# voidful/DeSTA2.5-Audio

Hardware: AMD Instinct MI355X
Metric: train steps/sec (node) Whisper-v3+Llama3.1-8B Q-Former6L at 1/2/4/8 MI355X (higher is better)
Workload: dtype bf16

## Files before the change

desta2.5-audio_amd/csrc/gemm_bf16.hip:

```cpp
#include "common.h"
#include "desta_hip.h"
#include <math.h>

#ifndef GEMM_GROUP_M
#define GEMM_GROUP_M 8
#endif

namespace {

typedef __attribute__((ext_vector_type(4))) unsigned u32x4;
typedef __attribute__((ext_vector_type(2))) float f32x2;

constexpr int BM = 128, BN = 128, BK = 64;
constexpr int TILE_BYTES = BM * BK * 2;

struct GemmArgs {
    const bf16_t* A; const bf16_t* B; void* C;
    int M, N, K;
    long lda, ldb, ldc;
    long sA, sB, sC;
    const float* bias;
    const void* res; long ldr; long sR; int res_f32;
    int act;
    int out_f32;
    bf16_t* preact; long ldp; long sP;
    float alpha;
    bf16_t* aux; long lda_x;
    unsigned drop_thresh, seed_lo, seed_hi; float drop_scale;
    int tilesM, tilesN;
    int full_tiles, split;
    union {
        float* ws;
        const float* b_scale;
    };
    int* tickets;
    const float* rms_w; float rms_eps;
    const float* rope_cs; const int* rope_pos; int rope_cols, rope_hd;
    int tail_skip;
};

__device__ __forceinline__ void rope4(const GemmArgs& p, int m, int n0, float (&v)[4]) {
    if (p.rope_cs && n0 < p.rope_cols) {
        const int pos = p.rope_pos[m];
        const float4 cs = *(const float4*)(p.rope_cs + ((long)pos * (p.rope_hd >> 1) + ((n0 & (p.rope_hd - 1)) >> 1)) * 2);
        const float a0 = v[0], b0 = v[1], a1 = v[2], b1 = v[3];
        v[0] = a0 * cs.x - b0 * cs.y; v[1] = b0 * cs.x + a0 * cs.y;
        v[2] = a1 * cs.z - b1 * cs.w; v[3] = b1 * cs.z + a1 * cs.w;
    }
}

__device__ __forceinline__ void gelu4_bf16(float (&v)[4]) {
#pragma unroll
    for (int e = 0; e < 4; ++e) v[e] = gelu_erf_fast(v[e]);
}

__device__ __forceinline__ void glds16(const void* g, void* l) {
    __builtin_amdgcn_global_load_lds((const __attribute__((address_space(1))) void*)g,
                                     (__attribute__((address_space(3))) void*)l, 16, 0, 0);
}

template <bool ROPE = false>
__device__ __forceinline__ void epilogue4(const GemmArgs& p, int z, int m, int n0, const f32x4& a) {
    float v[4];
#pragma unroll
    for (int e = 0; e < 4; ++e) v[e] = a[e] * p.alpha;
    if (p.bias) {
        const float4 b = *(const float4*)(p.bias + n0);
        v[0] += b.x; v[1] += b.y; v[2] += b.z; v[3] += b.w;
    }
    if constexpr (ROPE) rope4(p, m, n0, v);
    if (p.preact) {
        u16x4 o;
#pragma unroll
        for (int e = 0; e < 4; ++e) o[e] = f2bf(v[e]);
        *(u16x4*)(p.preact + (long)z * p.sP + (long)m * p.ldp + n0) = o;
    }
    if (p.act == 1) {
        if (p.out_f32) {
#pragma unroll
            for (int e = 0; e < 4; ++e) v[e] = gelu_erf(v[e]);
        } else {
            gelu4_bf16(v);
        }
    }
    if (p.drop_thresh) {
        const unsigned long base = ((unsigned long)z * p.M + m) * p.N + n0;
#pragma unroll
        for (int e = 0; e < 4; ++e) v[e] = desta_keep(p.seed_lo, p.seed_hi, base + e, p.drop_thresh) ? v[e] * p.drop_scale : 0.f;
    }
    if (p.res) {
        if (p.res_f32) {
            const float4 r = *(const float4*)((const float*)p.res + (long)z * p.sR + (long)m * p.ldr + n0);
            v[0] += r.x; v[1] += r.y; v[2] += r.z; v[3] += r.w;
        } else {
            const u16x4 r = *(const u16x4*)((const bf16_t*)p.res + (long)z * p.sR + (long)m * p.ldr + n0);
#pragma unroll
            for (int e = 0; e < 4; ++e) v[e] += bf2f(r[e]);
        }
    }
    if (p.out_f32) {
        *(float4*)((float*)p.C + (long)z * p.sC + (long)m * p.ldc + n0) = make_float4(v[0], v[1], v[2], v[3]);
    } else {
        u16x4 o;
#pragma unroll
        for (int e = 0; e < 4; ++e) o[e] = f2bf(v[e]);
        *(u16x4*)((bf16_t*)p.C + (long)z * p.sC + (long)m * p.ldc + n0) = o;
    }
}

__device__ __forceinline__ void epilogue4_f32_stream(const GemmArgs& p, int z, int m, int n0, const f32x4& a) {
    const float4 b = *(const float4*)(p.bias + n0);
    const float4 r = *(const float4*)((const float*)p.res + (long)z * p.sR + (long)m * p.ldr + n0);
    *(float4*)((float*)p.C + (long)z * p.sC + (long)m * p.ldc + n0) =
        make_float4((a[0] * p.alpha + b.x) + r.x, (a[1] * p.alpha + b.y) + r.y, (a[2] * p.alpha + b.z) + r.z, (a[3] * p.alpha + b.w) + r.w);
}

template <int MODE = -1>
__device__ __forceinline__ void epilogue_pair_bf16(const GemmArgs& p, int z, int m, bool row_ok, int ncol0, int fq,
                                                   const f32x4& a0, const f32x4& a1) {
    constexpr bool DYN = MODE < 0;
    const bool has_bias = DYN ? p.bias != nullptr : (MODE & 1) != 0;
    const bool has_gelu = DYN ? p.act == 1 : (MODE & 2) != 0;
    const bool has_rope = DYN ? true : (MODE & 4) != 0;
    const bool has_res = DYN ? p.res != nullptr : (MODE & 8) != 0;
    const bool has_pre = DYN ? p.preact != nullptr : (MODE & 16) != 0;
    if (has_res && !p.res_f32 && (p.ldr & 7) == 0 && (p.sR & 7) == 0) {
        float v[2][4];
#pragma unroll
        for (int t = 0; t < 2; ++t) {
            const f32x4& a = t ? a1 : a0;
            const int n0 = ncol0 + t * 16 + fq * 4;
#pragma unroll
            for (int e = 0; e < 4; ++e) v[t][e] = a[e] * p.alpha;
            if (has_bias) {
                const float4 b = *(const float4*)(p.bias + n0);
                v[t][0] += b.x; v[t][1] += b.y; v[t][2] += b.z; v[t][3] += b.w;
            }
            if (has_gelu) gelu4_bf16(v[t]);
        }
        const int col = ncol0 + (fq & 1) * 16 + (fq >> 1) * 8;
        const u16x8 r = *(const u16x8*)((const bf16_t*)p.res + (long)z * p.sR + (long)m * p.ldr + col);
        float w[8];
#pragma unroll
        for (int e = 0; e < 4; ++e) {
            const auto sw = __builtin_amdgcn_permlane16_swap(__float_as_uint(v[0][e]), __float_as_uint(v[1][e]), false, false);
            w[e] = __uint_as_float(sw[0]);
            w[4 + e] = __uint_as_float(sw[1]);
        }
        u16x8 o;
#pragma unroll
        for (int e = 0; e < 8; ++e) o[e] = f2bf(w[e] + bf2f(r[e]));
        if (row_ok) *(u16x8*)((bf16_t*)p.C + (long)z * p.sC + (long)m * p.ldc + col) = o;
        return;
    }
    unsigned pk[2][2];
#pragma unroll
    for (int t = 0; t < 2; ++t) {
        const f32x4& a = t ? a1 : a0;
        const int n0 = ncol0 + t * 16 + fq * 4;
        float v[4];
#pragma unroll
        for (int e = 0; e < 4; ++e) v[e] = a[e] * p.alpha;
        if (has_bias) {
            const float4 b = *(const float4*)(p.bias + n0);
            v[0] += b.x; v[1] += b.y; v[2] += b.z; v[3] += b.w;
        }
        if (has_rope) rope4(p, min(m, p.M - 1), n0, v);
        if (has_gelu) gelu4_bf16(v);
        if (has_res) {
            if (p.res_f32) {
                const float4 r = *(const float4*)((const float*)p.res + (long)z * p.sR + (long)m * p.ldr + n0);
                v[0] += r.x; v[1] += r.y; v[2] += r.z; v[3] += r.w;
            } else {
                const u16x4 r = *(const u16x4*)((const bf16_t*)p.res + (long)z * p.sR + (long)m * p.ldr + n0);
#pragma unroll
                for (int e = 0; e < 4; ++e) v[e] += bf2f(r[e]);
            }
        }
        pk[t][0] = (unsigned)f2bf(v[0]) | ((unsigned)f2bf(v[1]) << 16);
        pk[t][1] = (unsigned)f2bf(v[2]) | ((unsigned)f2bf(v[3]) << 16);
    }
    const auto lo = __builtin_amdgcn_permlane16_swap(pk[0][0], pk[1][0], false, false);
    const auto hi = __builtin_amdgcn_permlane16_swap(pk[0][1], pk[1][1], false, false);
    const int col = ncol0 + (fq & 1) * 16 + (fq >> 1) * 8;
    if (row_ok) {
        const uint4 o = make_uint4(lo[0], hi[0], lo[1], hi[1]);
        *(uint4*)((bf16_t*)p.C + (long)z * p.sC + (long)m * p.ldc + col) = o;
        if (has_pre) *(uint4*)(p.preact + (long)z * p.sP + (long)m * p.ldp + col) = o;
    }
}

__device__ __forceinline__ uint4 pair_swap_pk(unsigned x0, unsigned x1, unsigned y0, unsigned y1) {
    const auto lo = __builtin_amdgcn_permlane16_swap(x0, y0, false, false);
    const auto hi = __builtin_amdgcn_permlane16_swap(x1, y1, false, false);
    return make_uint4(lo[0], hi[0], lo[1], hi[1]);
}
__device__ __forceinline__ unsigned pk2(float a, float b) { return (unsigned)f2bf(a) | ((unsigned)f2bf(b) << 16); }

__device__ __forceinline__ void epilogue_swiglu_fwd(const GemmArgs& p, int z, int m, bool row_ok, int ncol0, int fq,
                                                    const f32x4& a0, const f32x4& a1, const f32x4& a2, const f32x4& a3) {
    float g[2][4], u[2][4], o[2][4];
#pragma unroll
    for (int e = 0; e < 4; ++e) {
        g[0][e] = bf2f(f2bf(a0[e] * p.alpha)); g[1][e] = bf2f(f2bf(a1[e] * p.alpha));
        u[0][e] = bf2f(f2bf(a2[e] * p.alpha)); u[1][e] = bf2f(f2bf(a3[e] * p.alpha));
    }
#pragma unroll
    for (int t = 0; t < 2; ++t)
#pragma unroll
        for (int e = 0; e < 4; ++e) {
            const float sg = g[t][e] / (1.0f + __expf(-g[t][e]));
            o[t][e] = bf2f(f2bf(sg)) * u[t][e];
        }
    const int col8 = (fq & 1) * 16 + (fq >> 1) * 8;
    const uint4 vg = pair_swap_pk(pk2(g[0][0], g[0][1]), pk2(g[0][2], g[0][3]), pk2(g[1][0], g[1][1]), pk2(g[1][2], g[1][3]));
    const uint4 vu = pair_swap_pk(pk2(u[0][0], u[0][1]), pk2(u[0][2], u[0][3]), pk2(u[1][0], u[1][1]), pk2(u[1][2], u[1][3]));
    const uint4 vo = pair_swap_pk(pk2(o[0][0], o[0][1]), pk2(o[0][2], o[0][3]), pk2(o[1][0], o[1][1]), pk2(o[1][2], o[1][3]));
    if (row_ok) {
        bf16_t* c = (bf16_t*)p.C + (long)z * p.sC + (long)m * p.ldc + ncol0 + col8;
        *(uint4*)c = vg;
        *(uint4*)(c + 32) = vu;
        *(uint4*)(p.aux + (long)m * p.lda_x + (ncol0 >> 1) + col8) = vo;
    }
}
__device__ __forceinline__ void epilogue_swiglu_bwd(const GemmArgs& p, int z, int m, bool row_ok, int ncol0, int fq,
                                                    const f32x4& a0, const f32x4& a1, const f32x4& a2, const f32x4& a3) {
    const int col8 = (fq & 1) * 16 + (fq >> 1) * 8;
#pragma unroll
    for (int h = 0; h < 2; ++h) {
        const f32x4& x = h ? a2 : a0;
        const f32x4& y = h ? a3 : a1;
        float d[8];
#pragma unroll
        for (int e = 0; e < 4; ++e) {
            const auto sw = __builtin_amdgcn_permlane16_swap(__float_as_uint(bf2f(f2bf(x[e] * p.alpha))), __float_as_uint(bf2f(f2bf(y[e] * p.alpha))), false, false);
            d[e] = __uint_as_float(sw[0]);
            d[4 + e] = __uint_as_float(sw[1]);
        }
        const long off = (long)m * p.lda_x + 2 * (ncol0 + 32 * h) + col8;
        const u16x8 gv = *(const u16x8*)(p.aux + off);
        const u16x8 uv = *(const u16x8*)(p.aux + off + 32);
        u16x8 og, ou;
#pragma unroll
        for (int e = 0; e < 8; ++e) {
            const float gg = bf2f(gv[e]), uu = bf2f(uv[e]);
            const float sig = 1.0f / (1.0f + __expf(-gg));
            const float sg = gg * sig;
            ou[e] = f2bf(d[e] * sg);
            og[e] = f2bf(d[e] * uu * (sig * (1.0f + gg * (1.0f - sig))));
        }
        if (row_ok) {
            bf16_t* c = (bf16_t*)p.C + (long)z * p.sC + (long)m * p.ldc + 2 * (ncol0 + 32 * h) + col8;
            *(u16x8*)c = og;
            *(u16x8*)(c + 32) = ou;
        }
    }
}

__device__ __forceinline__ int tr_swz(int k) { return (k & 3) | (((k >> 3) & 3) << 2); }
__device__ __forceinline__ bf16x8 frag_trans(const char* img, int out0, int kk, int fr, int fq) {
    typedef __attribute__((ext_vector_type(4))) __bf16 bf16x4_t;
    const int col = out0 + 4 * (fr & 3);
    bf16x8 o;
#pragma unroll
    for (int s2 = 0; s2 < 2; ++s2) {
        const int k = kk * 32 + 8 * fq + 4 * s2 + (fr >> 2);
        const int off = k * 256 + (((col >> 3) ^ tr_swz(k)) << 4) + ((col & 4) << 1);
        const bf16x4_t v = __builtin_amdgcn_ds_read_tr16_b64_v4bf16((__attribute__((address_space(3))) bf16x4_t*)(img + off));
        o[4 * s2 + 0] = v[0]; o[4 * s2 + 1] = v[1]; o[4 * s2 + 2] = v[2]; o[4 * s2 + 3] = v[3];
    }
    return o;
}

template <bool TA, bool TB>
__global__ __launch_bounds__(256, 2) void gemm_bf16_nt_kernel(GemmArgs p) {
    __shared__ __attribute__((aligned(16))) char lds[2 * 2 * TILE_BYTES];

    const int tid = threadIdx.x, lane = tid & 63, wave = tid >> 6;
    const int wr = wave >> 1, wc = wave & 1;

    const int ntile = p.tilesM * p.tilesN;
    const int L = xcd_remap(blockIdx.x, ntile);
    constexpr int GROUP_M = 8;
    const int gspan = GROUP_M * p.tilesN;
    const int first_m = (L / gspan) * GROUP_M;
    const int gsz = min(p.tilesM - first_m, GROUP_M);
    const int tm = first_m + (L % gspan) % gsz;
    const int tn = (L % gspan) / gsz;
    const int brow = tm * BM, bcol = tn * BN;
    const int z = blockIdx.y;

    const bf16_t* A = p.A + (long)z * p.sA;
    const bf16_t* B = p.B + (long)z * p.sB;

    const bf16_t* srcA[4];
    const bf16_t* srcB[4];
#pragma unroll
    for (int i = 0; i < 4; ++i) {
        const int idx = i * 256 + tid;
        if (TA) {
            const int k = idx >> 4, c = (idx & 15) ^ tr_swz(k);
            srcA[i] = A + (long)k * p.lda + min(brow + c * 8, p.M - 8);
        } else {
            const int r = idx >> 3, c = (idx & 7) ^ (r & 7);
            srcA[i] = A + (long)min(brow + r, p.M - 1) * p.lda + c * 8;
        }
        if (TB) {
            const int k = idx >> 4, c = (idx & 15) ^ tr_swz(k);
            srcB[i] = B + (long)k * p.ldb + min(bcol + c * 8, p.N - 8);
        } else {
            const int r = idx >> 3, c = (idx & 7) ^ (r & 7);
            srcB[i] = B + (long)min(bcol + r, p.N - 1) * p.ldb + c * 8;
        }
    }
    const long stepA = TA ? (long)BK * p.lda : BK, stepB = TB ? (long)BK * p.ldb : BK;
    auto stage = [&](int buf, int kt) {
        char* la = lds + buf * 2 * TILE_BYTES;
        char* lb = la + TILE_BYTES;
#pragma unroll
        for (int i = 0; i < 4; ++i) {
            const int wbase = (i * 256 + wave * 64) * 16;
            glds16(srcA[i] + kt * stepA, la + wbase);
            glds16(srcB[i] + kt * stepB, lb + wbase);
        }
    };

    f32x4 acc[4][4];
#pragma unroll
    for (int i = 0; i < 4; ++i)
#pragma unroll
        for (int j = 0; j < 4; ++j) acc[i][j] = f32x4{0.f, 0.f, 0.f, 0.f};

    const int fr = lane & 15, fq = lane >> 4;
    int offA[4], offB[4];
#pragma unroll
    for (int i = 0; i < 4; ++i) {
        const int ra = wr * 64 + i * 16 + fr;
        const int rb = wc * 64 + i * 16 + fr;
        offA[i] = ra * 128 + ((fq ^ (ra & 7)) << 4);
        offB[i] = rb * 128 + ((fq ^ (rb & 7)) << 4);
    }

    const int nk = p.K / BK;
    stage(0, 0);
    __syncthreads();
    for (int kt = 0; kt < nk; ++kt) {
        const int cur = kt & 1;
        if (kt + 1 < nk) stage(cur ^ 1, kt + 1);
        const char* la = lds + cur * 2 * TILE_BYTES;
        const char* lb = la + TILE_BYTES;
#pragma unroll
        for (int kk = 0; kk < 2; ++kk) {
            bf16x8 af[4], bfr[4];
#pragma unroll
            for (int i = 0; i < 4; ++i) {
                if (TA) af[i] = frag_trans(la, wr * 64 + i * 16, kk, fr, fq);
                else af[i] = *(const bf16x8*)(la + (offA[i] ^ (kk << 6)));
                if (TB) bfr[i] = frag_trans(lb, wc * 64 + i * 16, kk, fr, fq);
                else bfr[i] = *(const bf16x8*)(lb + (offB[i] ^ (kk << 6)));
            }
#pragma unroll
            for (int i = 0; i < 4; ++i)
#pragma unroll
                for (int j = 0; j < 4; ++j)
                    acc[i][j] = __builtin_amdgcn_mfma_f32_16x16x32_bf16(bfr[j], af[i], acc[i][j], 0, 0, 0);
        }
        __syncthreads();
    }

    if constexpr (!TA && !TB) {
        if (p.act == 2 || p.act == 3) {
            const int ncol0 = bcol + wc * 64;
            if (ncol0 < p.N) {
#pragma unroll
                for (int i = 0; i < 4; ++i) {
                    const int m = brow + wr * 64 + i * 16 + fr;
                    if (p.act == 2) epilogue_swiglu_fwd(p, z, min(m, p.M - 1), m < p.M, ncol0, fq, acc[i][0], acc[i][1], acc[i][2], acc[i][3]);
                    else epilogue_swiglu_bwd(p, z, min(m, p.M - 1), m < p.M, ncol0, fq, acc[i][0], acc[i][1], acc[i][2], acc[i][3]);
                }
            }
            return;
        }
    }
#pragma unroll
    for (int i = 0; i < 4; ++i) {
        const int m = brow + wr * 64 + i * 16 + fr;
        if (m >= p.M) continue;
#pragma unroll
        for (int j = 0; j < 4; ++j) {
            const int n0 = bcol + wc * 64 + j * 16 + fq * 4;
            if (n0 >= p.N) continue;
            epilogue4<true>(p, z, m, n0, acc[i][j]);
        }
    }
}


__device__ __forceinline__ bf16x8 frag_trans_raw(const char* img, int out0, int kk, int fr, int fq) {
    typedef __attribute__((ext_vector_type(4))) __bf16 bf16x4_t;
    const int col = out0 + 4 * (fr & 3);
    bf16x8 o;
#pragma unroll
    for (int s2 = 0; s2 < 2; ++s2) {
// ... 152 lines not shown
                __builtin_amdgcn_sched_group_barrier(0x100, 1, 0);
            }
        }
        __builtin_amdgcn_sched_barrier(0);
        landed(a0, b0);
    }
    asm volatile("s_waitcnt vmcnt(0)" ::: "memory");

    if constexpr (!TA && !TB) {
        if (p.act == 2 || p.act == 3) {
            const int ncol0 = bcol + wc * 64;
            if (ncol0 < p.N) {
#pragma unroll
                for (int i = 0; i < 4; ++i) {
                    const int m = brow + wr * 64 + i * 16 + fr;
                    if (p.act == 2) epilogue_swiglu_fwd(p, z, min(m, p.M - 1), m < p.M, ncol0, fq, acc[i][0], acc[i][1], acc[i][2], acc[i][3]);
                    else epilogue_swiglu_bwd(p, z, min(m, p.M - 1), m < p.M, ncol0, fq, acc[i][0], acc[i][1], acc[i][2], acc[i][3]);
                }
            }
            return;
        }
    }
#pragma unroll
    for (int i = 0; i < 4; ++i) {
        const int m = brow + wr * 64 + i * 16 + fr;
        if (m >= p.M) continue;
#pragma unroll
        for (int j = 0; j < 4; ++j) {
            const int n0 = bcol + wc * 64 + j * 16 + fq * 4;
            if (n0 >= p.N) continue;
            epilogue4<true>(p, z, m, n0, acc[i][j]);
        }
    }
}


constexpr int HT = 128 * BK * 2;

struct K256Stream {
    const bf16_t* src[4][2];
    char* lds;
    int kt0, nk, n_ht, wave;
    bool tskip;
    __device__ __forceinline__ void init(const GemmArgs& p, char* lds_, int tid, int wave_, const bf16_t* A, const bf16_t* B,
                                         int brow, int bcol, int kt0_, int nk_, bool tskip_) {
        lds = lds_; wave = wave_; kt0 = kt0_; nk = nk_; n_ht = 4 * nk_; tskip = tskip_;
#pragma unroll
        for (int i = 0; i < 2; ++i) {
            const int idx = i * 512 + tid;
            const int r = idx >> 3, pc = idx & 7;
            const int c = pc ^ (r & 7);
#pragma unroll
            for (int s2 = 0; s2 < 2; ++s2) {
                const int arow = (r >> 6) * 128 + s2 * 64 + (r & 63);
                const int bcolr = (r >> 5) * 64 + s2 * 32 + (r & 31);
                src[s2][i] = A + (long)min(brow + arow, p.M - 1) * p.lda + c * 8;
                src[2 + s2][i] = B + (long)min(bcol + bcolr, p.N - 1) * p.ldb + c * 8;
            }
        }
    }
    __device__ __forceinline__ void stage(int j) {
        if (tskip && j >= n_ht) return;
        const int t = j >> 2, q = j & 3;
        const int kind = (q == 0) ? 0 : (q == 1) ? 2 : (q == 2) ? 3 : 1;
        const long koff = (long)(kt0 + min(t, nk - 1)) * BK;
        char* dst = lds + ((t & 1) * 4 + kind) * HT;
#pragma unroll
        for (int i = 0; i < 2; ++i)
            glds16(src[kind][i] + koff, dst + (i * 512 + wave * 64) * 16);
    }
    __device__ __forceinline__ void stage_steady(int j) {
        const int t = j >> 2, q = j & 3;
        const int kind = (q == 0) ? 0 : (q == 1) ? 2 : (q == 2) ? 3 : 1;
        const long koff = (long)(kt0 + t) * BK;
        char* dst = lds + ((t & 1) * 4 + kind) * HT;
#pragma unroll
        for (int i = 0; i < 2; ++i)
            glds16(src[kind][i] + koff, dst + (i * 512 + wave * 64) * 16);
    }
    __device__ __forceinline__ void wait_steady(int) { asm volatile("s_waitcnt vmcnt(8)" ::: "memory"); }
    __device__ __forceinline__ void tail_wait(int issued) {
        const int ov = tskip ? issued - n_ht : 0;
        if (ov <= 0) asm volatile("s_waitcnt vmcnt(8)" ::: "memory");
        else if (ov == 1) asm volatile("s_waitcnt vmcnt(6)" ::: "memory");
        else if (ov == 2) asm volatile("s_waitcnt vmcnt(4)" ::: "memory");
        else if (ov == 3) asm volatile("s_waitcnt vmcnt(2)" ::: "memory");
        else asm volatile("s_waitcnt vmcnt(0)" ::: "memory");
    }
};

template <bool STAGGER, class AtTail>
__device__ __forceinline__ void k256_loop_2phase(K256Stream& st, const int (&offA)[4], const int (&offB)[2], f32x4 (&acc)[8][4],
                                                 AtTail&& at_tail) {
    const int nk = st.nk, wave = st.wave;
    const char* lds = st.lds;
    bf16x8 a[4][2], b0[2][2], b1[2][2];
#define MFMA_SLOT(ACC_I0, ACC_J0, BF)                                                                        \
    __builtin_amdgcn_sched_barrier(0);                                                                       \
    __builtin_amdgcn_s_setprio(1);                                                                           \
    _Pragma("unroll") for (int kk = 0; kk < 2; ++kk)                                                         \
        _Pragma("unroll") for (int i = 0; i < 4; ++i)                                                        \
            _Pragma("unroll") for (int j = 0; j < 2; ++j)                                                    \
                acc[ACC_I0 + i][ACC_J0 + j] =                                                                \
                    __builtin_amdgcn_mfma_f32_16x16x32_bf16(BF[j][kk], a[i][kk], acc[ACC_I0 + i][ACC_J0 + j], 0, 0, 0); \
    __builtin_amdgcn_s_setprio(0);                                                                           \
    __builtin_amdgcn_sched_barrier(0);
#define KTILE_2PHASE(STAGE, WAIT)                                                                              \
    {                                                                                                          \
        _Pragma("unroll") for (int i = 0; i < 2; ++i)                                                          \
            _Pragma("unroll") for (int kk = 0; kk < 2; ++kk) {                                                 \
                b0[i][kk] = *(const bf16x8*)(B0 + (offB[i] ^ (kk << 6)));                                      \
                b1[i][kk] = *(const bf16x8*)(B1 + (offB[i] ^ (kk << 6)));                                      \
            }                                                                                                  \
        _Pragma("unroll") for (int i = 0; i < 4; ++i)                                                          \
            _Pragma("unroll") for (int kk = 0; kk < 2; ++kk) a[i][kk] = *(const bf16x8*)(A0 + (offA[i] ^ (kk << 6))); \
        st.STAGE(g + 7);                                                                                       \
        asm volatile("s_waitcnt lgkmcnt(0)" ::: "memory");                                                     \
        if (STAGGER) { st.WAIT(g + 8); __builtin_amdgcn_s_barrier(); }                                         \
        MFMA_SLOT(0, 0, b0)                                                                                    \
        MFMA_SLOT(0, 2, b1)                                                                                    \
        st.WAIT(g + 8); __builtin_amdgcn_s_barrier();                                                          \
        _Pragma("unroll") for (int i = 0; i < 4; ++i)                                                          \
            _Pragma("unroll") for (int kk = 0; kk < 2; ++kk) a[i][kk] = *(const bf16x8*)(A1 + (offA[i] ^ (kk << 6))); \
        st.STAGE(g + 8);                                                                                       \
        st.STAGE(g + 9);                                                                                       \
        st.STAGE(g + 10);                                                                                      \
        asm volatile("s_waitcnt lgkmcnt(0)" ::: "memory");                                                     \
        if (STAGGER) { st.WAIT(g + 11); __builtin_amdgcn_s_barrier(); }                                       \
        MFMA_SLOT(4, 2, b1)                                                                                    \
        MFMA_SLOT(4, 0, b0)                                                                                    \
        st.WAIT(g + 11); __builtin_amdgcn_s_barrier();                                                         \
    }
    if (STAGGER && wave >= 4) __builtin_amdgcn_s_barrier();
    const int nk_steady = max(nk - 2, 0);
    for (int t = 0; t < nk_steady; ++t) {
        const char* base = lds + (t & 1) * 4 * HT;
        const char* A0 = base, *A1 = base + HT, *B0 = base + 2 * HT, *B1 = base + 3 * HT;
        const int g = 4 * t;
        KTILE_2PHASE(stage_steady, wait_steady)
    }
    at_tail();
    for (int t = nk_steady; t < nk; ++t) {
        const char* base = lds + (t & 1) * 4 * HT;
        const char* A0 = base, *A1 = base + HT, *B0 = base + 2 * HT, *B1 = base + 3 * HT;
        const int g = 4 * t;
        KTILE_2PHASE(stage, tail_wait)
    }
    if (STAGGER && wave < 4) __builtin_amdgcn_s_barrier();
#undef KTILE_2PHASE
#undef MFMA_SLOT
}

constexpr int E256_DYN = -2, E256_SWIGLU_FWD = 32, E256_SWIGLU_BWD = 33, E256_F32_STREAM = 64;
template <int EPI>
__device__ __forceinline__ void k256_epilogue(const GemmArgs& p, int z, int brow, int bcol, int wm, int wn, int fr, int fq,
                                              const f32x4 (&acc)[8][4]) {
    if constexpr (EPI == E256_SWIGLU_FWD || EPI == E256_SWIGLU_BWD) {
        const int ncol0 = bcol + wn * 64;
        if (ncol0 < p.N) {
#pragma unroll
            for (int i = 0; i < 8; ++i) {
                const int m = brow + wm * 128 + i * 16 + fr;
                if (EPI == E256_SWIGLU_FWD) epilogue_swiglu_fwd(p, z, min(m, p.M - 1), m < p.M, ncol0, fq, acc[i][0], acc[i][1], acc[i][2], acc[i][3]);
                else epilogue_swiglu_bwd(p, z, min(m, p.M - 1), m < p.M, ncol0, fq, acc[i][0], acc[i][1], acc[i][2], acc[i][3]);
            }
        }
        return;
    }
#define DESTA_WIDE_TILE(MODE)                                                                                          \
        _Pragma("unroll") for (int i = 0; i < 8; ++i) {                                                                \
            const int m = brow + wm * 128 + i * 16 + fr;                                                               \
            const int mc = min(m, p.M - 1);                                                                            \
            _Pragma("unroll") for (int j = 0; j < 4; j += 2) {                                                         \
                const int ncol0 = bcol + wn * 64 + j * 16;                                                             \
                if (ncol0 >= p.N) continue;                                                          \
                epilogue_pair_bf16<MODE>(p, z, mc, m < p.M, ncol0, fq, acc[i][j], acc[i][j + 1]);    \
            }                                                                                                          \
        }
#define DESTA_F32_STREAM_TILE()                                                                                        \
        _Pragma("unroll") for (int i = 0; i < 8; ++i) {                                                                \
            const int m = brow + wm * 128 + i * 16 + fr;                                                               \
            if (m >= p.M) continue;                                                                                    \
            _Pragma("unroll") for (int j = 0; j < 4; ++j) {                                                            \
                const int n0 = bcol + wn * 64 + j * 16 + fq * 4;                                                       \
                if (n0 >= p.N) continue;                                                                               \
                epilogue4_f32_stream(p, z, m, n0, acc[i][j]);                                                          \
            }                                                                                                          \
        }
    if constexpr (EPI == E256_F32_STREAM) {
        DESTA_F32_STREAM_TILE()
    } else if constexpr (EPI >= 0) {
        DESTA_WIDE_TILE(EPI)
    } else {
        const bool pre_ok = !p.preact || (p.act == 0 && !p.res && (p.ldp & 7) == 0 && (p.sP & 7) == 0);
        const bool wide = !p.out_f32 && pre_ok && p.act <= 1 && !p.drop_thresh && (p.N % 32 == 0) && (p.ldc % 8 == 0);
        if (wide) {
            DESTA_WIDE_TILE(-1)
            return;
        }
#pragma unroll
        for (int i = 0; i < 8; ++i) {
            const int m = brow + wm * 128 + i * 16 + fr;
            if (m >= p.M) continue;
#pragma unroll
            for (int j = 0; j < 4; ++j) {
                const int n0 = bcol + wn * 64 + j * 16 + fq * 4;
                if (n0 >= p.N) continue;
                epilogue4(p, z, m, n0, acc[i][j]);
            }
        }
    }
#undef DESTA_F32_STREAM_TILE
#undef DESTA_WIDE_TILE
}

__device__ __forceinline__ void k256_store_slab(float* slab, int wm, int wn, int fr, int fq, const f32x4 (&acc)[8][4]) {
#pragma unroll
    for (int i = 0; i < 8; ++i)
#pragma unroll
        for (int j = 0; j < 4; ++j)
            *(f32x4*)(slab + (wm * 128 + i * 16 + fr) * 256 + wn * 64 + j * 16 + fq * 4) = acc[i][j];
}

template <bool STAGGER, int PHASES, int EPI = 0>
__global__ __launch_bounds__(512, 2) void gemm_bf16_nt_256_kernel(GemmArgs p) {
    __shared__ __attribute__((aligned(16))) char lds[2 * 4 * HT];

    const int tid = threadIdx.x, lane = tid & 63, wave = __builtin_amdgcn_readfirstlane(tid >> 6);
    const int wm = wave >> 2, wn = wave & 3;

    int L, slice = 0;
    if ((int)blockIdx.x < p.full_tiles) {
        L = xcd_remap(blockIdx.x, p.full_tiles);
    } else {
        const int j = blockIdx.x - p.full_tiles;
        L = p.full_tiles + j / p.split;
        slice = j % p.split;
    }
    constexpr int GROUP_M = GEMM_GROUP_M;
    const int gspan = GROUP_M * p.tilesN;
    const int first_m = (L / gspan) * GROUP_M;
    const int gsz = min(p.tilesM - first_m, GROUP_M);
    const int tm = first_m + (L % gspan) % gsz;
    const int tn = (L % gspan) / gsz;
    const int brow = tm * 256, bcol = tn * 256;
    const int z = blockIdx.y;
    const bf16_t* A = p.A + (long)z * p.sA;
    const bf16_t* B = p.B + (long)z * p.sB;

    const int nk_all = p.K / BK;
    const bool partial = (int)blockIdx.x >= p.full_tiles && p.split > 1;
    const int kt0 = partial ? (int)((long)nk_all * slice / p.split) : 0;
    const int kt1 = partial ? (int)((long)nk_all * (slice + 1) / p.split) : nk_all;
    const int nk = kt1 - kt0;
    K256Stream st;
    st.init(p, lds, tid, wave, A, B, brow, bcol, kt0, nk, PHASES == 2 && p.tail_skip != 0);

    f32x4 acc[8][4];
#pragma unroll
    for (int i = 0; i < 8; ++i)
#pragma unroll
        for (int j = 0; j < 4; ++j) acc[i][j] = f32x4{0.f, 0.f, 0.f, 0.f};

    const int fr = lane & 15, fq = lane >> 4;
    int offA[4], offB[2];
#pragma unroll
    for (int i = 0; i < 4; ++i) {
        const int r = wm * 64 + i * 16 + fr;
        offA[i] = r * 128 + ((fq ^ (r & 7)) << 4);
    }
#pragma unroll
    for (int i = 0; i < 2; ++i) {
        const int r = wn * 32 + i * 16 + fr;
        offB[i] = r * 128 + ((fq ^ (r & 7)) << 4);
    }

#pragma unroll
    for (int j = 0; j < 7; ++j) st.stage(j);
    if (PHASES == 4) asm volatile("s_waitcnt vmcnt(10)" ::: "memory");
    else st.tail_wait(7);
    __builtin_amdgcn_s_barrier();

    if constexpr (PHASES == 2) {
        k256_loop_2phase<STAGGER>(st, offA, offB, acc, [] {});
    } else {
        bf16x8 a[4][2], b0[2][2], b1[2][2];
#define SLOT_END()                                                                                                  \
    asm volatile("s_waitcnt vmcnt(10)" ::: "memory");                                                               \
    __builtin_amdgcn_s_barrier();
#define MFMA_SLOT(ACC_I0, ACC_J0, BF)                                                                        \
    __builtin_amdgcn_sched_barrier(0);                                                                       \
    __builtin_amdgcn_s_setprio(1);                                                                           \
    _Pragma("unroll") for (int kk = 0; kk < 2; ++kk)                                                         \
        _Pragma("unroll") for (int i = 0; i < 4; ++i)                                                        \
            _Pragma("unroll") for (int j = 0; j < 2; ++j)                                                    \
                acc[ACC_I0 + i][ACC_J0 + j] =                                                                \
                    __builtin_amdgcn_mfma_f32_16x16x32_bf16(BF[j][kk], a[i][kk], acc[ACC_I0 + i][ACC_J0 + j], 0, 0, 0); \
    __builtin_amdgcn_s_setprio(0);                                                                           \
    __builtin_amdgcn_sched_barrier(0);
        if (STAGGER && wave >= 4) __builtin_amdgcn_s_barrier();
        for (int t = 0; t < nk; ++t) {
            const char* base = lds + (t & 1) * 4 * HT;
            const char* A0 = base, *A1 = base + HT, *B0 = base + 2 * HT, *B1 = base + 3 * HT;
            const int g = 4 * t;
#pragma unroll
            for (int i = 0; i < 2; ++i)
#pragma unroll
                for (int kk = 0; kk < 2; ++kk) b0[i][kk] = *(const bf16x8*)(B0 + (offB[i] ^ (kk << 6)));
#pragma unroll
            for (int i = 0; i < 4; ++i)
#pragma unroll
                for (int kk = 0; kk < 2; ++kk) a[i][kk] = *(const bf16x8*)(A0 + (offA[i] ^ (kk << 6)));
            st.stage(g + 7);
            asm volatile("s_waitcnt lgkmcnt(0)" ::: "memory");
            if (STAGGER) { SLOT_END() }
            MFMA_SLOT(0, 0, b0)
            SLOT_END()
#pragma unroll
            for (int i = 0; i < 2; ++i)
#pragma unroll
                for (int kk = 0; kk < 2; ++kk) b1[i][kk] = *(const bf16x8*)(B1 + (offB[i] ^ (kk << 6)));
            st.stage(g + 8);
            asm volatile("s_waitcnt lgkmcnt(0)" ::: "memory");
            if (STAGGER) { SLOT_END() }
            MFMA_SLOT(0, 2, b1)
            SLOT_END()
#pragma unroll
            for (int i = 0; i < 4; ++i)
#pragma unroll
                for (int kk = 0; kk < 2; ++kk) a[i][kk] = *(const bf16x8*)(A1 + (offA[i] ^ (kk << 6)));
            st.stage(g + 9);
            asm volatile("s_waitcnt lgkmcnt(0)" ::: "memory");
            if (STAGGER) { SLOT_END() }
            MFMA_SLOT(4, 2, b1)
            SLOT_END()
            st.stage(g + 10);
            if (STAGGER) { SLOT_END() }
            MFMA_SLOT(4, 0, b0)
            SLOT_END()
        }
        if (STAGGER && wave < 4) __builtin_amdgcn_s_barrier();
#undef MFMA_SLOT
#undef SLOT_END
    }
    asm volatile("s_waitcnt vmcnt(0)" ::: "memory");

    if (partial) {
        float* slab = p.ws + ((long)z * (p.tilesM * p.tilesN - p.full_tiles) * p.split +
                              (long)(blockIdx.x - p.full_tiles)) * (256 * 256);
        k256_store_slab(slab, wm, wn, fr, fq, acc);
        if (!p.tickets) return;
        __shared__ int s_go;
        int* tk = p.tickets + 2 * ((long)z * (p.tilesM * p.tilesN - p.full_tiles) + (L - p.full_tiles));
        asm volatile("s_waitcnt vmcnt(0)" ::: "memory");
        __syncthreads();
        if (tid == 0) {
            __builtin_amdgcn_fence(__ATOMIC_RELEASE, "agent");
            asm volatile("s_waitcnt vmcnt(0)" ::: "memory");
            __hip_atomic_fetch_add(tk, 1, __ATOMIC_RELAXED, __HIP_MEMORY_SCOPE_AGENT);
            int spins = 0, ok = 1;
            while (__hip_atomic_load(tk, __ATOMIC_RELAXED, __HIP_MEMORY_SCOPE_AGENT) < p.split) {
                __builtin_amdgcn_s_sleep(2);
                if (++spins > (1 << 21)) { ok = 0; break; }
            }
            __builtin_amdgcn_fence(__ATOMIC_ACQUIRE, "agent");
            asm volatile("s_waitcnt vmcnt(0)" ::: "memory");
            s_go = ok;
        }
        __syncthreads();
        if (s_go) {
            const float* s0 = p.ws + ((long)z * (p.tilesM * p.tilesN - p.full_tiles) + (L - p.full_tiles)) * p.split * (256 * 256);
            const int r0 = 256 * slice / p.split, r1 = 256 * (slice + 1) / p.split;
            for (int idx = tid; idx < (r1 - r0) * 64; idx += 512) {
                const int ml = r0 + (idx >> 6), nl = (idx & 63) * 4;
                const float* q = s0 + ml * 256 + nl;
                f32x4 v = *(const f32x4*)q;
                for (int s2 = 1; s2 < p.split; ++s2) {
                    const f32x4 w = *(const f32x4*)(q + (long)s2 * (256 * 256));
                    v[0] += w[0]; v[1] += w[1]; v[2] += w[2]; v[3] += w[3];
                }
                const int m = brow + ml, n0 = bcol + nl;
                if (m < p.M && n0 < p.N) epilogue4<true>(p, z, m, n0, v);
            }
        }
        __syncthreads();
        if (tid == 0) {
            const int dpt = __hip_atomic_fetch_add(tk + 1, 1, __ATOMIC_RELAXED, __HIP_MEMORY_SCOPE_AGENT);
            if (dpt == p.split - 1) {
                __hip_atomic_store(tk, 0, __ATOMIC_RELAXED, __HIP_MEMORY_SCOPE_AGENT);
                __hip_atomic_store(tk + 1, 0, __ATOMIC_RELAXED, __HIP_MEMORY_SCOPE_AGENT);
            }
        }
        return;
    }
    if constexpr (EPI == 1) {
        const int ncol0 = bcol + wn * 64;
        if (ncol0 < p.N) {
#pragma unroll
            for (int i = 0; i < 8; ++i) {
                const int m = brow + wm * 128 + i * 16 + fr;
                if (p.act == 2) epilogue_swiglu_fwd(p, z, min(m, p.M - 1), m < p.M, ncol0, fq, acc[i][0], acc[i][1], acc[i][2], acc[i][3]);
                else epilogue_swiglu_bwd(p, z, min(m, p.M - 1), m < p.M, ncol0, fq, acc[i][0], acc[i][1], acc[i][2], acc[i][3]);
            }
        }
        return;
    }
    const bool pre_ok = !p.preact || (p.act == 0 && !p.res && (p.ldp & 7) == 0 && (p.sP & 7) == 0);
    const bool wide = !p.out_f32 && pre_ok && p.act <= 1 && !p.drop_thresh && (p.N % 32 == 0) && (p.ldc % 8 == 0);
    if (wide) {
#define DESTA_WIDE_TILE(MODE)                                                                                          \
        _Pragma("unroll") for (int i = 0; i < 8; ++i) {                                                                \
            const int m = brow + wm * 128 + i * 16 + fr;                                                               \
            const int mc = min(m, p.M - 1);                                                                            \
            _Pragma("unroll") for (int j = 0; j < 4; j += 2) {                                                         \
                const int ncol0 = bcol + wn * 64 + j * 16;                                                             \
                if (ncol0 >= p.N) continue;                                                          \
                epilogue_pair_bf16<MODE>(p, z, mc, m < p.M, ncol0, fq, acc[i][j], acc[i][j + 1]);    \
            }                                                                                                          \
        }
        const int mode = (p.bias ? 1 : 0) | (p.act == 1 ? 2 : 0) | (p.rope_cs ? 4 : 0) | (p.res ? 8 : 0) | (p.preact ? 16 : 0);
        if (mode == 0) { DESTA_WIDE_TILE(0) }
        else if (mode == 8) { DESTA_WIDE_TILE(8) }
        else if (mode == 4) { DESTA_WIDE_TILE(4) }
        else if (mode == 1) { DESTA_WIDE_TILE(1) }
        else if (mode == 3) { DESTA_WIDE_TILE(3) }
        else if (mode == 16) { DESTA_WIDE_TILE(16) }
        else { DESTA_WIDE_TILE(-1) }
#undef DESTA_WIDE_TILE
        return;
    }
    if (p.out_f32 && p.bias && p.res && p.res_f32 && !p.preact && p.act == 0 && !p.drop_thresh) {
#pragma unroll
        for (int i = 0; i < 8; ++i) {
            const int m = brow + wm * 128 + i * 16 + fr;
            if (m >= p.M) continue;
#pragma unroll
            for (int j = 0; j < 4; ++j) {
                const int n0 = bcol + wn * 64 + j * 16 + fq * 4;
                if (n0 >= p.N) continue;
                epilogue4_f32_stream(p, z, m, n0, acc[i][j]);
            }
        }
        return;
    }
#pragma unroll
    for (int i = 0; i < 8; ++i) {
        const int m = brow + wm * 128 + i * 16 + fr;
        if (m >= p.M) continue;
#pragma unroll
        for (int j = 0; j < 4; ++j) {
            const int n0 = bcol + wn * 64 + j * 16 + fq * 4;
            if (n0 >= p.N) continue;
            epilogue4(p, z, m, n0, acc[i][j]);
        }
    }
}

template <int EPI>
__global__ __launch_bounds__(512, 2) void gemm_bf16_nt_256p_kernel(GemmArgs p, int* queue) {
    __shared__ __attribute__((aligned(16))) char lds[2 * 4 * HT + 16];
    int* s_ticket = (int*)(lds + 2 * 4 * HT);
    const int tid = threadIdx.x, lane = tid & 63, wave = __builtin_amdgcn_readfirstlane(tid >> 6);
    const int wm = wave >> 2, wn = wave & 3;
    const int fr = lane & 15, fq = lane >> 4;
    constexpr int GROUP_M = GEMM_GROUP_M;
    const int nk_all = p.K / BK;

    const int xq = blockIdx.x & 7;
    const int F = p.full_tiles, q8 = F >> 3, r8 = F & 7;
    const int lo = (xq < r8) ? xq * (q8 + 1) : r8 * (q8 + 1) + (xq - r8) * q8;
    const int n_full = q8 + (xq < r8 ? 1 : 0);
    const int n_split_items = p.split > 1 ? (p.tilesM * p.tilesN - F) * p.split : 0;
    const int n_items = n_full + (n_split_items > xq ? (n_split_items - xq + 7) >> 3 : 0);
    int* counter = queue + xq;

    int brow, bcol, kt0, nk, slab;
    bool partial;
    auto geometry = [&](int tk) {
        int L, slice = 0;
        partial = tk >= n_full;
        if (!partial) {
            L = lo + tk;
        } else {
            slab = xq + 8 * (tk - n_full);
            L = F + slab / p.split;
            slice = slab % p.split;
        }
        const int gspan = GROUP_M * p.tilesN;
        const int first_m = (L / gspan) * GROUP_M;
        const int gsz = min(p.tilesM - first_m, GROUP_M);
        brow = (first_m + (L % gspan) % gsz) * 256;
        bcol = ((L % gspan) / gsz) * 256;
        kt0 = partial ? (int)((long)nk_all * slice / p.split) : 0;
        const int kt1 = partial ? (int)((long)nk_all * (slice + 1) / p.split) : nk_all;
        nk = kt1 - kt0;
    };
    auto draw = [&]() { return __hip_atomic_fetch_add(counter, 1, __ATOMIC_RELAXED, __HIP_MEMORY_SCOPE_AGENT); };

    int offA[4], offB[2];
#pragma unroll
    for (int i = 0; i < 4; ++i) {
        const int r = wm * 64 + i * 16 + fr;
        offA[i] = r * 128 + ((fq ^ (r & 7)) << 4);
    }
#pragma unroll
    for (int i = 0; i < 2; ++i) {
        const int r = wn * 32 + i * 16 + fr;
        offB[i] = r * 128 + ((fq ^ (r & 7)) << 4);
    }

    if (tid == 0) *s_ticket = draw();
    __syncthreads();
    int tk = *s_ticket;
    K256Stream st;
    if (tk < n_items) {
        geometry(tk);
        st.init(p, lds, tid, wave, p.A, p.B, brow, bcol, kt0, nk, p.tail_skip != 0);
#pragma unroll
        for (int j = 0; j < 7; ++j) st.stage(j);
    }
    f32x4 acc[8][4];
    while (tk < n_items) {
#pragma unroll
        for (int i = 0; i < 8; ++i)
#pragma unroll
            for (int j = 0; j < 4; ++j) acc[i][j] = f32x4{0.f, 0.f, 0.f, 0.f};
        st.tail_wait(7);
        __builtin_amdgcn_s_barrier();
        int nxt;
        k256_loop_2phase<true>(st, offA, offB, acc, [&] {
            const unsigned lane_mask = __builtin_amdgcn_readfirstlane(wave == 0 ? 1u : 0u);
            unsigned long saved;
            asm volatile("s_mov_b64 %1, exec\n\t"
                         "s_mov_b32 exec_lo, %3\n\t"
                         "s_mov_b32 exec_hi, 0\n\t"
                         "global_atomic_add %0, %2, %4, off sc0\n\t"
                         "s_mov_b64 exec, %1"
                         : "=&v"(nxt), "=&s"(saved) : "v"(counter), "s"(lane_mask), "v"(1) : "memory");
        });
        asm volatile("s_waitcnt vmcnt(0)" ::: "memory");
        if (tid == 0) *s_ticket = nxt;
        __syncthreads();
        const int cur_brow = brow, cur_bcol = bcol, cur_slab = slab;
        const bool cur_partial = partial;
        tk = *s_ticket;
        if (tk < n_items) {
            geometry(tk);
            st.init(p, lds, tid, wave, p.A, p.B, brow, bcol, kt0, nk, p.tail_skip != 0);
#pragma unroll
            for (int j = 0; j < 7; ++j) st.stage(j);
        }
        if constexpr (EPI != E256_SWIGLU_FWD && EPI != E256_SWIGLU_BWD) {
            if (cur_partial) {
                k256_store_slab(p.ws + (long)cur_slab * (256 * 256), wm, wn, fr, fq, acc);
                continue;
            }
        }
        k256_epilogue<EPI>(p, 0, cur_brow, cur_bcol, wm, wn, fr, fq, acc);
    }
    asm volatile("s_waitcnt vmcnt(0)" ::: "memory");
    __syncthreads();
    if (tid == 0) {
        const int dpt = __hip_atomic_fetch_add(queue + 8, 1, __ATOMIC_RELAXED, __HIP_MEMORY_SCOPE_AGENT);
        if (dpt == (int)gridDim.x - 1) {
#pragma unroll
            for (int k = 0; k < 9; ++k) __hip_atomic_store(queue + k, 0, __ATOMIC_RELAXED, __HIP_MEMORY_SCOPE_AGENT);
        }
    }
}

__global__ __launch_bounds__(256) void gemm_splitk_fixup_kernel(GemmArgs p) {
    const int rem = p.tilesM * p.tilesN - p.full_tiles;
    const int ti = blockIdx.x / 64, part = blockIdx.x % 64;
    const int z = blockIdx.y;
    const int L = p.full_tiles + ti;
    constexpr int GROUP_M = GEMM_GROUP_M;
    const int gspan = GROUP_M * p.tilesN;
    const int first_m = (L / gspan) * GROUP_M;
    const int gsz = min(p.tilesM - first_m, GROUP_M);
    const int tm = first_m + (L % gspan) % gsz;
    const int tn = (L % gspan) / gsz;
    const int ml = part * 4 + (threadIdx.x >> 6), nl = (threadIdx.x & 63) * 4;
    const float* slab = p.ws + ((long)z * rem + ti) * p.split * (256 * 256) + ml * 256 + nl;
    f32x4 acc = *(const f32x4*)slab;
    for (int s2 = 1; s2 < p.split; ++s2) {
        const f32x4 v = *(const f32x4*)(slab + (long)s2 * (256 * 256));
        acc[0] += v[0]; acc[1] += v[1]; acc[2] += v[2]; acc[3] += v[3];
    }
    const int m = tm * 256 + ml, n0 = tn * 256 + nl;
    if (m < p.M && n0 < p.N) epilogue4<true>(p, z, m, n0, acc);
}

template <int COLS, int U, bool W8>
struct SkinnyStage {
    bf16x8 w0[U][COLS / 16], w1[U][COLS / 16], x0[U], x1[U];
};
template <int COLS, int U>
// ... 649 lines not shown
```

Measured before the change: 6.522.

## Software-pipeline GEMM epilogue side-loads for interior tiles with batched prefetch

Adds a batched epilogue path for fully interior tiles that prefetches bias, RoPE positions and tables, residual rows, or SwiGLU aux data several rows ahead of use. Loads overlap with the epilogue math and stores of earlier rows instead of stalling on each global load. It also pins parts of the RoPE rotation with inline asm to steer FMA scheduling. The cost is more register pressure and more code, plus a second epilogue path that must stay numerically consistent with the guarded path.

Result: no change. 6.546 (median of 6 runs) (+0.4%).

```diff
diff --git a/desta2.5-audio_amd/csrc/gemm_bf16.hip b/desta2.5-audio_amd/csrc/gemm_bf16.hip
--- a/desta2.5-audio_amd/csrc/gemm_bf16.hip
+++ b/desta2.5-audio_amd/csrc/gemm_bf16.hip
@@ -39,13 +39,27 @@
     int tail_skip;
 };
 
+__device__ __forceinline__ void rope4_rot(const float4 cs, float (&v)[4]) {
+    const float a0 = v[0], b0 = v[1], a1 = v[2], b1 = v[3];
+    v[0] = a0 * cs.x - b0 * cs.y; v[1] = b0 * cs.x + a0 * cs.y;
+    v[2] = a1 * cs.z - b1 * cs.w; v[3] = b1 * cs.z + a1 * cs.w;
+}
+__device__ __forceinline__ void rope4_rot_pinned(const float4 cs, float (&v)[4]) {
+    const float a0 = v[0], b0 = v[1], a1 = v[2], b1 = v[3];
+    float p0 = a0 * cs.x, q0 = b0 * cs.y, r0 = b0 * cs.x, q1 = b1 * cs.w, r1 = a1 * cs.w;
+    asm("" : "+v"(p0), "+v"(q0), "+v"(r0), "+v"(q1), "+v"(r1));
+    v[0] = p0 - q0;
+    v[1] = __builtin_fmaf(a0, cs.y, r0);
+    v[2] = __builtin_fmaf(a1, cs.z, -q1);
+    v[3] = __builtin_fmaf(b1, cs.z, r1);
+}
+template <bool PINNED = false>
 __device__ __forceinline__ void rope4(const GemmArgs& p, int m, int n0, float (&v)[4]) {
     if (p.rope_cs && n0 < p.rope_cols) {
         const int pos = p.rope_pos[m];
         const float4 cs = *(const float4*)(p.rope_cs + ((long)pos * (p.rope_hd >> 1) + ((n0 & (p.rope_hd - 1)) >> 1)) * 2);
-        const float a0 = v[0], b0 = v[1], a1 = v[2], b1 = v[3];
-        v[0] = a0 * cs.x - b0 * cs.y; v[1] = b0 * cs.x + a0 * cs.y;
-        v[2] = a1 * cs.z - b1 * cs.w; v[3] = b1 * cs.z + a1 * cs.w;
+        if constexpr (PINNED) rope4_rot_pinned(cs, v);
+        else rope4_rot(cs, v);
     }
 }
 
@@ -165,7 +179,7 @@
             const float4 b = *(const float4*)(p.bias + n0);
             v[0] += b.x; v[1] += b.y; v[2] += b.z; v[3] += b.w;
         }
-        if (has_rope) rope4(p, min(m, p.M - 1), n0, v);
+        if (has_rope) rope4<true>(p, min(m, p.M - 1), n0, v);
         if (has_gelu) gelu4_bf16(v);
         if (has_res) {
             if (p.res_f32) {
@@ -223,32 +237,34 @@
         *(uint4*)(p.aux + (long)m * p.lda_x + (ncol0 >> 1) + col8) = vo;
     }
 }
+__device__ __forceinline__ void swiglu_bwd_block(float alpha, const f32x4& x, const f32x4& y, const u16x8 gv, const u16x8 uv,
+                                                 u16x8& og, u16x8& ou) {
+    float d[8];
+#pragma unroll
+    for (int e = 0; e < 4; ++e) {
+        const auto sw = __builtin_amdgcn_permlane16_swap(__float_as_uint(bf2f(f2bf(x[e] * alpha))), __float_as_uint(bf2f(f2bf(y[e] * alpha))), false, false);
+        d[e] = __uint_as_float(sw[0]);
+        d[4 + e] = __uint_as_float(sw[1]);
+    }
+#pragma unroll
+    for (int e = 0; e < 8; ++e) {
+        const float gg = bf2f(gv[e]), uu = bf2f(uv[e]);
+        const float sig = 1.0f / (1.0f + __expf(-gg));
+        const float sg = gg * sig;
+        ou[e] = f2bf(d[e] * sg);
+        og[e] = f2bf(d[e] * uu * (sig * (1.0f + gg * (1.0f - sig))));
+    }
+}
 __device__ __forceinline__ void epilogue_swiglu_bwd(const GemmArgs& p, int z, int m, bool row_ok, int ncol0, int fq,
                                                     const f32x4& a0, const f32x4& a1, const f32x4& a2, const f32x4& a3) {
     const int col8 = (fq & 1) * 16 + (fq >> 1) * 8;
 #pragma unroll
     for (int h = 0; h < 2; ++h) {
-        const f32x4& x = h ? a2 : a0;
-        const f32x4& y = h ? a3 : a1;
-        float d[8];
-#pragma unroll
-        for (int e = 0; e < 4; ++e) {
-            const auto sw = __builtin_amdgcn_permlane16_swap(__float_as_uint(bf2f(f2bf(x[e] * p.alpha))), __float_as_uint(bf2f(f2bf(y[e] * p.alpha))), false, false);
-            d[e] = __uint_as_float(sw[0]);
-            d[4 + e] = __uint_as_float(sw[1]);
-        }
         const long off = (long)m * p.lda_x + 2 * (ncol0 + 32 * h) + col8;
         const u16x8 gv = *(const u16x8*)(p.aux + off);
         const u16x8 uv = *(const u16x8*)(p.aux + off + 32);
         u16x8 og, ou;
-#pragma unroll
-        for (int e = 0; e < 8; ++e) {
-            const float gg = bf2f(gv[e]), uu = bf2f(uv[e]);
-            const float sig = 1.0f / (1.0f + __expf(-gg));
-            const float sg = gg * sig;
-            ou[e] = f2bf(d[e] * sg);
-            og[e] = f2bf(d[e] * uu * (sig * (1.0f + gg * (1.0f - sig))));
-        }
+        swiglu_bwd_block(p.alpha, h ? a2 : a0, h ? a3 : a1, gv, uv, og, ou);
         if (row_ok) {
             bf16_t* c = (bf16_t*)p.C + (long)z * p.sC + (long)m * p.ldc + 2 * (ncol0 + 32 * h) + col8;
             *(u16x8*)c = og;
@@ -707,9 +723,187 @@
 }
 
 constexpr int E256_DYN = -2, E256_SWIGLU_FWD = 32, E256_SWIGLU_BWD = 33, E256_F32_STREAM = 64;
+
+struct EpiBatch { uint4 q[4]; };
+template <int EPI> struct EpiKind {
+    static constexpr bool bwd = EPI == E256_SWIGLU_BWD, f32s = EPI == E256_F32_STREAM, wide = EPI >= 0 && EPI < 32;
+    static constexpr bool res = wide && (EPI & 8) != 0, rope = wide && (EPI & 4) != 0, bias = f32s || (wide && (EPI & 1) != 0);
+    static constexpr bool loads = bwd || f32s || res || rope;
+    static constexpr bool any = loads || bias;
+    static constexpr int ahead = !loads ? 0 : res ? 4 : 2;
+    static_assert(!wide || !any || (EPI & 16) == 0, "no pre-activation copy in the batched forms");
+};
+template <int EPI> struct EpiPre {
+    float4 bias[4];
+    int pos[8];
+    EpiBatch b[EpiKind<EPI>::ahead > 0 ? EpiKind<EPI>::ahead : 1];
+    long lo, so;
+};
+__device__ __forceinline__ void k256_epi_pin(long& x) { asm volatile("" : "+v"(x)); }
+__device__ __forceinline__ void k256_epi_pin(float& x) { asm volatile("" : "+s"(x)); }
+template <int EPI> __device__ __forceinline__ const char* k256_epi_ld_base(const GemmArgs& p) {
+    return EpiKind<EPI>::bwd ? (const char*)p.aux : (const char*)p.res;
+}
+template <int EPI> __device__ __forceinline__ long k256_epi_ld_step(const GemmArgs& p) {
+    return EpiKind<EPI>::f32s ? p.ldr * 64 : EpiKind<EPI>::res ? p.ldr * 32 : EpiKind<EPI>::bwd ? p.lda_x * 32 : 0;
+}
+template <int EPI> __device__ __forceinline__ long k256_epi_st_step(const GemmArgs& p) { return EpiKind<EPI>::f32s ? p.ldc * 64 : p.ldc * 32; }
+template <int EPI>
+__device__ __forceinline__ bool k256_epi_interior(const GemmArgs& p, int brow, int bcol, int wm, int wn) {
+    if constexpr (!EpiKind<EPI>::any) return false;
+    bool ok = brow + wm * 128 + 128 <= p.M && bcol + wn * 64 + 64 <= p.N;
+    if constexpr (EpiKind<EPI>::res) ok = ok && !p.res_f32 && (p.ldr & 7) == 0 && (p.sR & 7) == 0;
+    return ok;
+}
+template <int EPI>
+__device__ __forceinline__ EpiBatch k256_epi_load(const GemmArgs& p, long lo, int pos, int ncol, int fq) {
+    EpiBatch b = {};
+    const char* lp = k256_epi_ld_base<EPI>(p) + lo;
+    if constexpr (EpiKind<EPI>::f32s) {
+#pragma unroll
+        for (int j = 0; j < 4; ++j) b.q[j] = *(const uint4*)(lp + j * 64);
+    } else if constexpr (EpiKind<EPI>::res) {
+#pragma unroll
+        for (int jp = 0; jp < 2; ++jp) b.q[jp] = *(const uint4*)(lp + jp * 64);
+    } else if constexpr (EpiKind<EPI>::rope) {
+#pragma unroll
+        for (int j = 0; j < 4; ++j) {
+            const int n0 = ncol + j * 16 + fq * 4;
+            b.q[j] = *(const uint4*)(p.rope_cs + ((long)pos * (p.rope_hd >> 1) + ((n0 & (p.rope_hd - 1)) >> 1)) * 2);
+        }
+    } else if constexpr (EpiKind<EPI>::bwd) {
+#pragma unroll
+        for (int h = 0; h < 4; ++h) b.q[h] = *(const uint4*)(lp + h * 64);
+    }
+    return b;
+}
+template <int EPI>
+__device__ __forceinline__ void k256_epi_prefetch(const GemmArgs& p, int z, int brow, int bcol, int wm, int wn, int fr, int fq,
+                                                  EpiPre<EPI>& pre) {
+    const int m0 = brow + wm * 128 + fr, ncol = bcol + wn * 64, col8 = (fq & 1) * 16 + (fq >> 1) * 8;
+    if constexpr (EpiKind<EPI>::f32s) {
+        pre.lo = 4 * ((long)z * p.sR + (long)m0 * p.ldr + ncol + fq * 4);
+        pre.so = 4 * ((long)z * p.sC + (long)m0 * p.ldc + ncol + fq * 4);
+    } else if constexpr (EpiKind<EPI>::bwd) {
+        pre.lo = 2 * ((long)m0 * p.lda_x + 2 * ncol + col8);
+        pre.so = 2 * ((long)z * p.sC + (long)m0 * p.ldc + 2 * ncol + col8);
+    } else {
+        pre.lo = EpiKind<EPI>::res ? 2 * ((long)z * p.sR + (long)m0 * p.ldr + ncol + col8) : 0;
+        pre.so = 2 * ((long)z * p.sC + (long)m0 * p.ldc + ncol + col8);
+    }
+    if constexpr (EpiKind<EPI>::bias) {
+#pragma unroll
+        for (int j = 0; j < 4; ++j) pre.bias[j] = *(const float4*)(p.bias + ncol + j * 16 + fq * 4);
+    }
+    if constexpr (EpiKind<EPI>::rope) {
+#pragma unroll
+        for (int i = 0; i < 8; ++i) pre.pos[i] = p.rope_pos[m0 + i * 16];
+    }
+#pragma unroll
+    for (int i = 0; i < EpiKind<EPI>::ahead; ++i) {
+        pre.b[i] = k256_epi_load<EPI>(p, pre.lo, EpiKind<EPI>::rope ? pre.pos[i] : 0, ncol, fq);
+        pre.lo += k256_epi_ld_step<EPI>(p);
+    }
+    __builtin_amdgcn_s_waitcnt(0);
+}
+template <int MODE>
+__device__ __forceinline__ void epilogue_pair_bf16_ops(float alpha, char* c, const f32x4& a0, const f32x4& a1,
+                                                       const float4& b0, const float4& b1, const uint4& q0, const uint4& q1, bool rope_on) {
+    float v[2][4];
+#pragma unroll
+    for (int t = 0; t < 2; ++t) {
+        const f32x4& a = t ? a1 : a0;
+        const float4& b = t ? b1 : b0;
+#pragma unroll
+        for (int e = 0; e < 4; ++e) v[t][e] = a[e] * alpha;
+        if constexpr ((MODE & 1) != 0) { v[t][0] += b.x; v[t][1] += b.y; v[t][2] += b.z; v[t][3] += b.w; }
+        if constexpr ((MODE & 4) != 0) {
+            float w[4] = {v[t][0], v[t][1], v[t][2], v[t][3]};
+            rope4_rot_pinned(__builtin_bit_cast(float4, t ? q1 : q0), w);
+#pragma unroll
+            for (int e = 0; e < 4; ++e) v[t][e] = rope_on ? w[e] : v[t][e];
+        }
+        if constexpr ((MODE & 2) != 0) gelu4_bf16(v[t]);
+    }
+    if constexpr ((MODE & 8) != 0) {
+        const u16x8 r = __builtin_bit_cast(u16x8, q0);
+        float w[8];
+#pragma unroll
+        for (int e = 0; e < 4; ++e) {
+            const auto sw = __builtin_amdgcn_permlane16_swap(__float_as_uint(v[0][e]), __float_as_uint(v[1][e]), false, false);
+            w[e] = __uint_as_float(sw[0]);
+            w[4 + e] = __uint_as_float(sw[1]);
+        }
+        u16x8 o;
+#pragma unroll
+        for (int e = 0; e < 8; ++e) o[e] = f2bf(w[e] + bf2f(r[e]));
+        *(u16x8*)c = o;
+    } else {
+        *(uint4*)c = pair_swap_pk(pk2(v[0][0], v[0][1]), pk2(v[0][2], v[0][3]), pk2(v[1][0], v[1][1]), pk2(v[1][2], v[1][3]));
+    }
+}
+template <int EPI>
+__device__ __forceinline__ void k256_epi_finish(const GemmArgs& p, float alpha, long so, int ncol, const f32x4 (&a)[4], const EpiBatch& cur,
+                                                const float4 (&bias)[4]) {
+    char* sp = (char*)p.C + so;
+    if constexpr (EpiKind<EPI>::f32s) {
+#pragma unroll
+        for (int j = 0; j < 4; ++j) {
+            const float4 r = __builtin_bit_cast(float4, cur.q[j]);
+            const float4 b = bias[j];
+            *(float4*)(sp + j * 64) = make_float4((a[j][0] * alpha + b.x) + r.x, (a[j][1] * alpha + b.y) + r.y,
+                                                  (a[j][2] * alpha + b.z) + r.z, (a[j][3] * alpha + b.w) + r.w);
+        }
+    } else if constexpr (EpiKind<EPI>::bwd) {
+#pragma unroll
+        for (int h = 0; h < 2; ++h) {
+            u16x8 og, ou;
+            swiglu_bwd_block(alpha, a[2 * h], a[2 * h + 1], __builtin_bit_cast(u16x8, cur.q[2 * h]), __builtin_bit_cast(u16x8, cur.q[2 * h + 1]), og, ou);
+            *(u16x8*)(sp + 128 * h) = og;
+            *(u16x8*)(sp + 128 * h + 64) = ou;
+        }
+    } else {
+#pragma unroll
+        for (int jp = 0; jp < 2; ++jp)
+            epilogue_pair_bf16_ops<EPI>(alpha, sp + jp * 64, a[2 * jp], a[2 * jp + 1], bias[2 * jp], bias[2 * jp + 1],
+                                        cur.q[EpiKind<EPI>::rope ? 2 * jp : jp], cur.q[2 * jp + 1],
+                                        EpiKind<EPI>::rope && ncol + jp * 32 < p.rope_cols);
+    }
+}
+template <int EPI>
+__device__ __forceinline__ void k256_epilogue_interior(const GemmArgs& p, int bcol, int wn, int fq, const f32x4 (&acc)[8][4], EpiPre<EPI>& pre) {
+    constexpr int AH = EpiKind<EPI>::ahead;
+    const int ncol = bcol + wn * 64;
+#pragma unroll
+    for (int i = 0; i < 8; ++i) {
+        EpiBatch cur = {};
+        if constexpr (AH > 0) {
+            cur = pre.b[i % AH];
+            if (i + AH < 8) {
+                k256_epi_pin(pre.lo);
+                pre.b[i % AH] = k256_epi_load<EPI>(p, pre.lo, EpiKind<EPI>::rope ? pre.pos[(i + AH) & 7] : 0, ncol, fq);
+                pre.lo += k256_epi_ld_step<EPI>(p);
+            }
+            __builtin_amdgcn_sched_barrier(0);
+        }
+        float alpha = p.alpha;
+        k256_epi_pin(alpha);
+        k256_epi_pin(pre.so);
+        k256_epi_finish<EPI>(p, alpha, pre.so, ncol, acc[i], cur, pre.bias);
+        pre.so += k256_epi_st_step<EPI>(p);
+    }
+}
 template <int EPI>
 __device__ __forceinline__ void k256_epilogue(const GemmArgs& p, int z, int brow, int bcol, int wm, int wn, int fr, int fq,
                                               const f32x4 (&acc)[8][4]) {
+    if constexpr (EpiKind<EPI>::any) {
+        if (k256_epi_interior<EPI>(p, brow, bcol, wm, wn)) {
+            EpiPre<EPI> pre;
+            k256_epi_prefetch<EPI>(p, z, brow, bcol, wm, wn, fr, fq, pre);
+            k256_epilogue_interior<EPI>(p, bcol, wn, fq, acc, pre);
+            return;
+        }
+    }
     if constexpr (EPI == E256_SWIGLU_FWD || EPI == E256_SWIGLU_BWD) {
         const int ncol0 = bcol + wn * 64;
         if (ncol0 < p.N) {
@@ -948,8 +1142,20 @@
         }
         return;
     }
+#define DESTA_BATCHED_TILE(E_, GUARDED)                                                                                \
+        if (k256_epi_interior<E_>(p, brow, bcol, wm, wn)) {                                                            \
+            EpiPre<E_> pre;                                                                                            \
+            k256_epi_prefetch<E_>(p, z, brow, bcol, wm, wn, fr, fq, pre);                                              \
+            k256_epilogue_interior<E_>(p, bcol, wn, fq, acc, pre);                                           \
+        } else { GUARDED }
     if constexpr (EPI == 1) {
         const int ncol0 = bcol + wn * 64;
+        if (p.act == 3 && k256_epi_interior<E256_SWIGLU_BWD>(p, brow, bcol, wm, wn)) {
+            EpiPre<E256_SWIGLU_BWD> pre;
+            k256_epi_prefetch<E256_SWIGLU_BWD>(p, z, brow, bcol, wm, wn, fr, fq, pre);
+            k256_epilogue_interior<E256_SWIGLU_BWD>(p, bcol, wn, fq, acc, pre);
+            return;
+        }
         if (ncol0 < p.N) {
 #pragma unroll
             for (int i = 0; i < 8; ++i) {
@@ -975,29 +1181,29 @@
         }
         const int mode = (p.bias ? 1 : 0) | (p.act == 1 ? 2 : 0) | (p.rope_cs ? 4 : 0) | (p.res ? 8 : 0) | (p.preact ? 16 : 0);
         if (mode == 0) { DESTA_WIDE_TILE(0) }
-        else if (mode == 8) { DESTA_WIDE_TILE(8) }
-        else if (mode == 4) { DESTA_WIDE_TILE(4) }
-        else if (mode == 1) { DESTA_WIDE_TILE(1) }
-        else if (mode == 3) { DESTA_WIDE_TILE(3) }
+        else if (mode == 8) { DESTA_BATCHED_TILE(8, DESTA_WIDE_TILE(8)) }
+        else if (mode == 4) { DESTA_BATCHED_TILE(4, DESTA_WIDE_TILE(4)) }
+        else if (mode == 1) { DESTA_BATCHED_TILE(1, DESTA_WIDE_TILE(1)) }
+        else if (mode == 3) { DESTA_BATCHED_TILE(3, DESTA_WIDE_TILE(3)) }
         else if (mode == 16) { DESTA_WIDE_TILE(16) }
         else { DESTA_WIDE_TILE(-1) }
 #undef DESTA_WIDE_TILE
         return;
     }
     if (p.out_f32 && p.bias && p.res && p.res_f32 && !p.preact && p.act == 0 && !p.drop_thresh) {
-#pragma unroll
-        for (int i = 0; i < 8; ++i) {
-            const int m = brow + wm * 128 + i * 16 + fr;
-            if (m >= p.M) continue;
-#pragma unroll
-            for (int j = 0; j < 4; ++j) {
-                const int n0 = bcol + wn * 64 + j * 16 + fq * 4;
-                if (n0 >= p.N) continue;
-                epilogue4_f32_stream(p, z, m, n0, acc[i][j]);
-            }
-        }
+        DESTA_BATCHED_TILE(E256_F32_STREAM,
+            _Pragma("unroll") for (int i = 0; i < 8; ++i) {
+                const int m = brow + wm * 128 + i * 16 + fr;
+                if (m >= p.M) continue;
+                _Pragma("unroll") for (int j = 0; j < 4; ++j) {
+                    const int n0 = bcol + wn * 64 + j * 16 + fq * 4;
+                    if (n0 >= p.N) continue;
+                    epilogue4_f32_stream(p, z, m, n0, acc[i][j]);
+                }
+            })
         return;
     }
+#undef DESTA_BATCHED_TILE
 #pragma unroll
     for (int i = 0; i < 8; ++i) {
         const int m = brow + wm * 128 + i * 16 + fr;
```
